# jiean001/MakeupDiffuse

Hardware: NVIDIA B200
Metric: DDIM-50 makeup images/sec at 256^2 (higher is better)
Workload: dtype bf16

## Files before the change

makeupdiffuse_b200/csrc/attention_tcgen05.cu:

```cuda
#include <cuda.h>
#include <stdlib.h>

#include "tcgen05.cuh"
using namespace mkd;
using namespace mkd::tc;

namespace {

constexpr int BQ = 128, BKV = 128;
constexpr int CH = 128 * 128;

template <int DN, int NWG_, int KST_, int VST_> struct ACfg {
  static constexpr int DCH = (DN + 63) / 64;
  static constexpr int NWG = NWG_, KST = KST_, VST = VST_;
  static constexpr int OSTR = (DN + 31) / 32 * 32;
  static constexpr int TCOLS = NWG * 128 + NWG * OSTR <= 256 ? 256 : 512;
  static constexpr int THREADS = 32 * (4 * NWG + 2);
  static constexpr int NBAR = 5 * NWG + 2 * KST + 2 * VST;
  static constexpr size_t SMEM = (size_t)(NWG * DCH + (KST + VST) * DCH + 2 * NWG) * CH + NBAR * 8 + 16;
  static_assert(NWG * 128 + NWG * OSTR <= 512, "TMEM columns");
  static_assert(SMEM <= 227 * 1024, "shared memory");
};

template <int DN, int NWG_, int KST_, int VST_>
__global__ void __launch_bounds__(ACfg<DN, NWG_, KST_, VST_>::THREADS, ACfg<DN, NWG_, KST_, VST_>::TCOLS == 256 ? 2 : 1)
    attn_tcgen05_kernel(const __grid_constant__ CUtensorMap qmap, const __grid_constant__ CUtensorMap kmap,
                        const __grid_constant__ CUtensorMap vmap, bf16* __restrict__ o, int Nq, int Nkv, int d, int ldo,
                        float sl2) {
  using C = ACfg<DN, NWG_, KST_, VST_>;
  constexpr int DCH = C::DCH, NWG = C::NWG, KST = C::KST, VST = C::VST;
  extern __shared__ __align__(1024) unsigned char smem_raw[];
  unsigned char* smem = smem_raw;
  if ((smem_u32(smem_raw) & 1023u) != 0) __trap();
  unsigned char* Qs = smem;
  unsigned char* Ks = Qs + NWG * DCH * CH;
  unsigned char* Vs = Ks + KST * DCH * CH;
  unsigned char* Ps = Vs + VST * DCH * CH;
  uint64_t* q_full = reinterpret_cast<uint64_t*>(Ps + NWG * 2 * CH);
  uint64_t* s_full = q_full + NWG;
  uint64_t* s_free = s_full + NWG;
  uint64_t* p_full = s_free + NWG;
  uint64_t* o_full = p_full + NWG;
  uint64_t* k_full = o_full + NWG;
  uint64_t* k_empty = k_full + KST;
  uint64_t* v_full = k_empty + KST;
  uint64_t* v_empty = v_full + VST;
  uint32_t* tmem_slot = reinterpret_cast<uint32_t*>(v_empty + VST);

  const int warp = threadIdx.x >> 5, lane = threadIdx.x & 31;
  constexpr int W_PROD = 4 * NWG, W_MMA = 4 * NWG + 1;
  const int b = blockIdx.z, h = blockIdx.y, q0 = blockIdx.x * (BQ * NWG);
  const int T = (Nkv + BKV - 1) / BKV;
  const int nwg = (NWG == 2 && q0 + BQ < Nq) ? 2 : 1;

  if (threadIdx.x == 0) {
    prefetch_tensormap(&qmap);
    prefetch_tensormap(&kmap);
    prefetch_tensormap(&vmap);
    for (int i = 0; i < NWG; ++i) {
      mbar_init(q_full + i, 1);
      mbar_init(s_full + i, 1);
      mbar_init(s_free + i, 4);
      mbar_init(p_full + i, 4);
      mbar_init(o_full + i, 1);
    }
    for (int i = 0; i < KST; ++i) {
      mbar_init(k_full + i, 1);
      mbar_init(k_empty + i, 1);
    }
    for (int i = 0; i < VST; ++i) {
      mbar_init(v_full + i, 1);
      mbar_init(v_empty + i, 1);
    }
    fence_barrier_init();
  }
  if (warp == W_MMA) tmem_alloc<C::TCOLS>(tmem_slot);
  fence_before();
  __syncthreads();
  fence_after();
  const uint32_t tmem_base = *tmem_slot;
  pdl_wait();
  if (warp == W_PROD) {
    if (lane == 0) {
      for (int wg = 0; wg < nwg; ++wg) {
        mbar_expect_tx(q_full + wg, DCH * CH);
        for (int c = 0; c < DCH; ++c) tma_load_4d(&qmap, q_full + wg, Qs + (wg * DCH + c) * CH, c * 64, h, q0 + wg * BQ, b);
      }
      for (int t = 0; t < T; ++t) {
        const int ks = t % KST, vs = t % VST;
        if (t >= KST) mbar_wait(k_empty + ks, (t / KST - 1) & 1);
        mbar_expect_tx(k_full + ks, DCH * CH);
        for (int c = 0; c < DCH; ++c) tma_load_4d(&kmap, k_full + ks, Ks + (ks * DCH + c) * CH, c * 64, h, t * BKV, b);
        if (t >= VST) mbar_wait(v_empty + vs, (t / VST - 1) & 1);
        mbar_expect_tx(v_full + vs, DCH * CH);
        for (int c = 0; c < DCH; ++c) tma_load_4d(&vmap, v_full + vs, Vs + (vs * DCH + c) * CH, c * 64, h, t * BKV, b);
      }
    }
  } else if (warp == W_MMA) {
    if (lane == 0) {
      constexpr uint32_t idesc_s = idesc_bf16(BQ, BKV, false);
      constexpr uint32_t idesc_o = idesc_bf16(BQ, DN, true);
      const int ksteps = (d + 15) >> 4;
      auto issue_s = [&](int wg, int st) {
        const uint32_t a = smem_u32(Qs + wg * DCH * CH), bk = smem_u32(Ks + st * DCH * CH);
        for (int ks = 0; ks < ksteps; ++ks) {
          const uint32_t off = (uint32_t)(ks >> 2) * CH + (uint32_t)(ks & 3) * 32;
          mma_bf16_ss(tmem_base + (uint32_t)(wg * BKV), smem_desc_sw128(a + off), smem_desc_sw128(bk + off), idesc_s, ks > 0);
        }
      };
      auto issue_pv = [&](int wg, int st, int kvalid, bool accumulate) {
        const uint32_t a = smem_u32(Ps + wg * 2 * CH), bv = smem_u32(Vs + st * DCH * CH);
        const int steps = (min(kvalid, BKV) + 15) >> 4;
        for (int kk = 0; kk < steps; ++kk) {
          const uint32_t aoff = (uint32_t)(kk >> 2) * CH + (uint32_t)(kk & 3) * 32;
          mma_bf16_ss(tmem_base + (uint32_t)(NWG * BKV + wg * C::OSTR), smem_desc_sw128(a + aoff),
                      smem_desc_sw128(bv + (uint32_t)kk * 2048, CH), idesc_o, accumulate || kk > 0);
        }
      };
      for (int wg = 0; wg < nwg; ++wg) mbar_wait(q_full + wg, 0);
      mbar_wait(k_full + 0, 0);
      fence_after();
      for (int wg = 0; wg < nwg; ++wg) {
        issue_s(wg, 0);
        commit(s_full + wg);
      }
      commit(k_empty + 0);
      for (int t = 0; t < T; ++t) {
        const int st = t % VST;
        if (t + 1 < T) {
          const int st1 = (t + 1) % KST;
          mbar_wait(k_full + st1, ((t + 1) / KST) & 1);
          for (int wg = 0; wg < nwg; ++wg) {
            mbar_wait(s_free + wg, t & 1);
            fence_after();
            issue_s(wg, st1);
            commit(s_full + wg);
          }
          commit(k_empty + st1);
        }
        mbar_wait(v_full + st, (t / VST) & 1);
        for (int wg = 0; wg < nwg; ++wg) {
          mbar_wait(p_full + wg, t & 1);
          fence_after();
          issue_pv(wg, st, Nkv - t * BKV, t > 0);
          commit(o_full + wg);
        }
        commit(v_empty + st);
      }
    }
  } else if ((warp >> 2) < nwg) {
    const int wg = warp >> 2, row = (warp & 3) * 32 + lane;
    const uint32_t lane_base = (uint32_t)((warp & 3) * 32) << 16;
    const uint32_t tS = tmem_base + lane_base + (uint32_t)(wg * BKV);
    const uint32_t tO = tmem_base + lane_base + (uint32_t)(NWG * BKV + wg * C::OSTR);
    unsigned char* Pw = Ps + wg * 2 * CH + row * 128;
    const uint32_t swz = (uint32_t)(row & 7);
    float m_used = -INFINITY, l = 0.f;

    for (int t = 0; t < T; ++t) {
      mbar_wait(s_full + wg, t & 1);
      fence_after();
      const int kvalid = Nkv - t * BKV;
      uint32_t v[4][32];
#pragma unroll
      for (int c = 0; c < 4; ++c) tmem_ld32_nowait(tS + c * 32, v[c]);
      tmem_ld_wait();
      fence_before();
      __syncwarp();
      if (lane == 0) mbar_arrive(s_free + wg);
      if (kvalid < BKV) {
#pragma unroll
        for (int c = 0; c < 4; ++c) {
#pragma unroll
          for (int i = 0; i < 32; ++i) v[c][i] = (c * 32 + i >= kvalid) ? 0xff800000u : v[c][i];
        }
      }
      float mx8[8];
#pragma unroll
      for (int i = 0; i < 8; ++i) mx8[i] = -INFINITY;
#pragma unroll
      for (int c = 0; c < 4; ++c) {
#pragma unroll
        for (int i = 0; i < 32; i += 2) mx8[(i >> 1) & 7] = max3(mx8[(i >> 1) & 7], __uint_as_float(v[c][i]), __uint_as_float(v[c][i + 1]));
      }
      const float mx = fmaxf(max3(mx8[0], mx8[1], mx8[2]), max3(mx8[3], mx8[4], fmaxf(max3(mx8[5], mx8[6], mx8[7]), -INFINITY)));
      if (t > 0) {
        mbar_wait(o_full + wg, (t - 1) & 1);
        fence_after();
      }
      if (__any_sync(0xffffffffu, (mx - m_used) * sl2 > 8.0f)) {
        const float m_new = fmaxf(m_used, mx);
        const float corr = ex2((m_used - m_new) * sl2);
        l *= corr;
        m_used = m_new;
        if (t > 0) {
#pragma unroll
          for (int g = 0; g < DN / 16; ++g) {
            uint32_t r[16];
            tmem_ld16_nowait(tO + g * 16, r);
            tmem_ld_wait();
#pragma unroll
            for (int i = 0; i < 16; ++i) r[i] = __float_as_uint(__uint_as_float(r[i]) * corr);
            tmem_st16(tO + g * 16, r);
          }
          tmem_st_wait();
        }
      }
      const float mb = m_used * sl2;
      const uint64_t sl2x2 = pack2(sl2, sl2), nmbx2 = pack2(-mb, -mb);
      uint64_t sum2[4] = {pack2(0.f, 0.f), pack2(0.f, 0.f), pack2(0.f, 0.f), pack2(0.f, 0.f)};
#pragma unroll
      for (int c = 0; c < 4; ++c) {
        uint32_t pk[16];
#pragma unroll
        for (int i = 0; i < 32; i += 2) {
          float a0, a1;
          unpack2(ffma2(pack2(__uint_as_float(v[c][i]), __uint_as_float(v[c][i + 1])), sl2x2, nmbx2), a0, a1);
          const float p0 = ex2(a0), p1 = ex2(a1);
          sum2[(i >> 1) & 3] = fadd2(sum2[(i >> 1) & 3], pack2(p0, p1));
          __nv_bfloat162 hh = __floats2bfloat162_rn(p0, p1);
          pk[i >> 1] = *reinterpret_cast<uint32_t*>(&hh);
        }
#pragma unroll
        for (int jj = 0; jj < 4; ++jj) {
          const uint32_t u = (uint32_t)(c * 4 + jj);
          unsigned char* dst = Pw + (u >> 3) * CH + (((u & 7) ^ swz) << 4);
          *reinterpret_cast<uint4*>(dst) = make_uint4(pk[4 * jj], pk[4 * jj + 1], pk[4 * jj + 2], pk[4 * jj + 3]);
        }
      }
      {
        float s0, s1, s2, s3;
        unpack2(fadd2(sum2[0], sum2[1]), s0, s1);
        unpack2(fadd2(sum2[2], sum2[3]), s2, s3);
        l += (s0 + s1) + (s2 + s3);
      }
      fence_before();
      fence_proxy_async_smem();
      __syncwarp();
      if (lane == 0) mbar_arrive(p_full + wg);
    }
    mbar_wait(o_full + wg, (T - 1) & 1);
    fence_after();
    const int q = q0 + wg * BQ + row;
    const float inv = 1.0f / l;
    bf16* dst = o + ((int64_t)b * Nq + q) * ldo + h * d;
#pragma unroll
    for (int g = 0; g < DN / 16; ++g) {
      uint32_t r[16];
      tmem_ld16_nowait(tO + g * 16, r);
      tmem_ld_wait();
#pragma unroll
      for (int hlf = 0; hlf < 2; ++hlf) {
        if (q < Nq && g * 16 + hlf * 8 < d) {
          float f[8];
#pragma unroll
          for (int i = 0; i < 8; ++i) f[i] = __uint_as_float(r[hlf * 8 + i]) * inv;
          store8(dst + g * 16 + hlf * 8, f);
        }
      }
    }
  }
  fence_before();
  __syncthreads();
  if (warp == W_MMA) {
    fence_after();
    tmem_dealloc<C::TCOLS>(tmem_base);
  }
}

constexpr int HKV = 64;
constexpr int HB = HKV * 128;

template <int DN>
__global__ void __launch_bounds__(320, 2)
    attn_split_kernel(const __grid_constant__ CUtensorMap qmap, const __grid_constant__ CUtensorMap kmap,
                      const __grid_constant__ CUtensorMap vmap, bf16* __restrict__ o, int Nq, int Nkv, int d, int ldo, float sl2) {
  static_assert(DN % 16 == 0 && DN <= 64, "one 64-channel chunk per head");
  constexpr int TCOLS = 256;
  extern __shared__ __align__(1024) unsigned char smem_raw[];
  unsigned char* smem = smem_raw;
  if ((smem_u32(smem_raw) & 1023u) != 0) __trap();
  unsigned char* Qs = smem;
  unsigned char* Ks = Qs + CH;
  unsigned char* Vs = Ks + 4 * HB;
  unsigned char* Ps = Vs + 4 * HB;
  uint64_t* q_full = reinterpret_cast<uint64_t*>(Ps + 2 * CH);
  uint64_t* s_full = q_full + 1;
  uint64_t* s_free = s_full + 2;
  uint64_t* p_full = s_free + 2;
  uint64_t* pv_done = p_full + 2;
  uint64_t* k_full = pv_done + 2;
  uint64_t* v_full = k_full + 4;
  uint32_t* tmem_slot = reinterpret_cast<uint32_t*>(v_full + 4);

  const int warp = threadIdx.x >> 5, lane = threadIdx.x & 31;
  constexpr int W_ISSUE = 8;
  const int b = blockIdx.z, h = blockIdx.y, q0 = blockIdx.x * BQ;
  const int H = (Nkv + HKV - 1) / HKV;

  if (threadIdx.x == 0) {
    prefetch_tensormap(&qmap);
    prefetch_tensormap(&kmap);
    prefetch_tensormap(&vmap);
    mbar_init(q_full, 1);
    for (int i = 0; i < 2; ++i) {
      mbar_init(s_full + i, 1);
      mbar_init(s_free + i, 4);
      mbar_init(p_full + i, 4);
      mbar_init(pv_done + i, 1);
    }
    for (int i = 0; i < 4; ++i) {
      mbar_init(k_full + i, 1);
      mbar_init(v_full + i, 1);
    }
    fence_barrier_init();
  }
  if (warp == W_ISSUE) tmem_alloc<TCOLS>(tmem_slot);
  fence_before();
  __syncthreads();
  fence_after();
  const uint32_t tmem_base = *tmem_slot;
  pdl_wait();
  if (warp >= W_ISSUE) {
    const int g = warp - W_ISSUE;
    const int n = (H - g + 1) >> 1;
    constexpr uint32_t idesc_s = idesc_bf16(BQ, HKV, false);
    constexpr uint32_t idesc_o = idesc_bf16(BQ, DN, true);
    constexpr int KS = DN / 16;
    unsigned char* Kg = Ks + g * 2 * HB;
    unsigned char* Vg = Vs + g * 2 * HB;
    const uint64_t qdesc = smem_desc_sw128(smem_u32(Qs));
    const uint64_t kdesc0 = smem_desc_sw128(smem_u32(Kg));
    const uint64_t vdesc0 = smem_desc_sw128(smem_u32(Vg), CH);
    const uint64_t pdesc = smem_desc_sw128(smem_u32(Ps + g * CH));
    const uint32_t dS = tmem_base + (uint32_t)(g * HKV), dO = tmem_base + (uint32_t)(2 * HKV + g * 64);
    auto load_k = [&](int u) {
      if (elect_one()) {
        mbar_expect_tx(k_full + 2 * g + (u & 1), HB);
        tma_load_4d(&kmap, k_full + 2 * g + (u & 1), Kg + (u & 1) * HB, 0, h, (g + 2 * u) * HKV, b);
      }
      __syncwarp();
    };
    auto load_v = [&](int u) {
      if (elect_one()) {
        mbar_expect_tx(v_full + 2 * g + (u & 1), HB);
        tma_load_4d(&vmap, v_full + 2 * g + (u & 1), Vg + (u & 1) * HB, 0, h, (g + 2 * u) * HKV, b);
      }
      __syncwarp();
    };
    auto issue_s = [&](int u) {
      mbar_wait(k_full + 2 * g + (u & 1), (u >> 1) & 1);
      fence_after();
      if (elect_one()) {
        const uint64_t kd = kdesc0 + (uint64_t)((u & 1) * (HB >> 4));
#pragma unroll
        for (int ks = 0; ks < KS; ++ks) mma_bf16_ss(dS, qdesc + (uint64_t)(ks * 2), kd + (uint64_t)(ks * 2), idesc_s, ks > 0);
        commit(s_full + g);
      }
      __syncwarp();
    };
    if (n > 0) {
      if (g == 0 && elect_one()) {
        mbar_expect_tx(q_full, CH);
        tma_load_4d(&qmap, q_full, Qs, 0, h, q0, b);
      }
      __syncwarp();
      load_k(0);
      load_v(0);
      if (n > 1) {
        load_k(1);
        load_v(1);
      }
      mbar_wait(q_full, 0);
      issue_s(0);
      for (int u = 0; u < n; ++u) {
        const int s = u & 1;
        if (u + 1 < n) {
          mbar_wait(s_free + g, u & 1);
          if (u + 2 < n) load_k(u + 2);
          issue_s(u + 1);
        }
        mbar_wait(v_full + 2 * g + s, (u >> 1) & 1);
        mbar_wait(p_full + g, u & 1);
        fence_after();
        if (u >= 1 && u + 1 < n) load_v(u + 1);
        if (elect_one()) {
          const uint64_t vd = vdesc0 + (uint64_t)(s * (HB >> 4));
          const int kvalid = Nkv - (g + 2 * u) * HKV;
          if (kvalid >= HKV) {
#pragma unroll
            for (int kk = 0; kk < 4; ++kk) mma_bf16_ss(dO, pdesc + (uint64_t)(kk * 2), vd + (uint64_t)(kk * 128), idesc_o, u > 0 || kk > 0);
          } else {
            const int steps = (kvalid + 15) >> 4;
            for (int kk = 0; kk < steps; ++kk) mma_bf16_ss(dO, pdesc + (uint64_t)(kk * 2), vd + (uint64_t)(kk * 128), idesc_o, u > 0 || kk > 0);
          }
          commit(pv_done + g);
        }
        __syncwarp();
      }
    }
  } else {
    const int g = warp >> 2, row = (warp & 3) * 32 + lane;
    const uint32_t lane_base = (uint32_t)((warp & 3) * 32) << 16;
    const uint32_t tS = tmem_base + lane_base + (uint32_t)(g * HKV);
    const uint32_t tO = tmem_base + lane_base + (uint32_t)(2 * HKV + g * 64);
    const uint32_t pw = smem_u32(Ps + g * CH + row * 128) + (((uint32_t)row & 7u) << 4);
    float m_used = -INFINITY, l = 0.f;
    int u = 0;
    for (int hh = g; hh < H; hh += 2, ++u) {
      mbar_wait(s_full + g, u & 1);
      fence_after();
      uint32_t v[2][32];
      tmem_ld32_nowait(tS, v[0]);
      tmem_ld32_nowait(tS + 32, v[1]);
      tmem_ld_wait();
      fence_before();
      __syncwarp();
      if (lane == 0) mbar_arrive(s_free + g);
      const int kvalid = Nkv - hh * HKV;
      if (kvalid < HKV) {
#pragma unroll
        for (int c = 0; c < 2; ++c) {
#pragma unroll
          for (int i = 0; i < 32; ++i) v[c][i] = (c * 32 + i >= kvalid) ? 0xff800000u : v[c][i];
        }
      }
      float mx8[8];
#pragma unroll
      for (int i = 0; i < 8; ++i) mx8[i] = -INFINITY;
#pragma unroll
      for (int c = 0; c < 2; ++c) {
#pragma unroll
        for (int i = 0; i < 32; i += 2) mx8[(i >> 1) & 7] = max3(mx8[(i >> 1) & 7], __uint_as_float(v[c][i]), __uint_as_float(v[c][i + 1]));
      }
      const float mx = fmaxf(max3(mx8[0], mx8[1], mx8[2]), max3(mx8[3], mx8[4], max3(mx8[5], mx8[6], mx8[7])));
      if (__any_sync(0xffffffffu, (mx - m_used) * sl2 > 8.0f)) {
        const float m_new = fmaxf(m_used, mx);
        const float corr = ex2((m_used - m_new) * sl2);
        l *= corr;
        m_used = m_new;
        if (u > 0) {
          mbar_wait(pv_done + g, (u - 1) & 1);
          fence_after();
#pragma unroll
          for (int gg = 0; gg < DN / 16; ++gg) {
            uint32_t r[16];
            tmem_ld16_nowait(tO + gg * 16, r);
            tmem_ld_wait();
#pragma unroll
            for (int i = 0; i < 16; ++i) r[i] = __float_as_uint(__uint_as_float(r[i]) * corr);
            tmem_st16(tO + gg * 16, r);
          }
          tmem_st_wait();
        }
      }
      const float mb = m_used * sl2;
      const uint64_t sl2x2 = pack2(sl2, sl2), nmbx2 = pack2(-mb, -mb);
      uint64_t sum2[4] = {pack2(0.f, 0.f), pack2(0.f, 0.f), pack2(0.f, 0.f), pack2(0.f, 0.f)};
      uint32_t pk[2][16];
#pragma unroll
      for (int c = 0; c < 2; ++c) {
#pragma unroll
        for (int i = 0; i < 32; i += 2) {
          float a0, a1;
          unpack2(ffma2(pack2(__uint_as_float(v[c][i]), __uint_as_float(v[c][i + 1])), sl2x2, nmbx2), a0, a1);
          const float p0 = ex2(a0), p1 = ex2(a1);
          sum2[(i >> 1) & 3] = fadd2(sum2[(i >> 1) & 3], pack2(p0, p1));
          __nv_bfloat162 hh2 = __floats2bfloat162_rn(p0, p1);
          pk[c][i >> 1] = *reinterpret_cast<uint32_t*>(&hh2);
        }
      }
      if (u > 0) {
        mbar_wait(pv_done + g, (u - 1) & 1);
        fence_after();
      }
#pragma unroll
      for (int c = 0; c < 2; ++c) {
#pragma unroll
        for (int jj = 0; jj < 4; ++jj)
          asm volatile("st.shared.v4.b32 [%0], {%1, %2, %3, %4};\n" ::"r"(pw ^ ((uint32_t)(c * 4 + jj) << 4)), "r"(pk[c][4 * jj]),
                       "r"(pk[c][4 * jj + 1]), "r"(pk[c][4 * jj + 2]), "r"(pk[c][4 * jj + 3])
                       : "memory");
      }
      {
        float s0, s1, s2, s3;
        unpack2(fadd2(sum2[0], sum2[1]), s0, s1);
        unpack2(fadd2(sum2[2], sum2[3]), s2, s3);
        l += (s0 + s1) + (s2 + s3);
      }
      fence_before();
      fence_proxy_async_smem();
      __syncwarp();
      if (lane == 0) mbar_arrive(p_full + g);
    }
    const bool two = H > 1;
    float2* ml = reinterpret_cast<float2*>(Ps);
    if (u > 0) {
      mbar_wait(pv_done + g, (u - 1) & 1);
      ml[g * (CH / 8) + row] = make_float2(m_used, l);
    }
    fence_before();
    asm volatile("bar.sync 1, 256;\n" ::: "memory");
    fence_after();
    const float2 mo = (g == 0 && !two) ? make_float2(-INFINITY, 0.f) : ml[(g ^ 1) * (CH / 8) + row];
    const float m = fmaxf(m_used, mo.x);
    const float a_own = ex2((m_used - m) * sl2), a_oth = ex2((mo.x - m) * sl2);
    const float inv = 1.0f / (l * a_own + mo.y * a_oth);
    const float c_own = a_own * inv, c_oth = a_oth * inv;
    const uint32_t tO_oth = tmem_base + lane_base + (uint32_t)(2 * HKV + (g ^ 1) * 64);
    const int q = q0 + row;
    bf16* dst = o + ((int64_t)b * Nq + q) * ldo + h * d;
#pragma unroll
    for (int gg = 0; gg < DN / 16; ++gg) {
      if ((gg & 1) != g) continue;
      uint32_t r0[16], r1[16];
      if (g == 0 || two) tmem_ld16_nowait(tO + gg * 16, r0);
      if (g == 1 || two) tmem_ld16_nowait(tO_oth + gg * 16, r1);
      tmem_ld_wait();
#pragma unroll
      for (int hlf = 0; hlf < 2; ++hlf) {
        if (q < Nq && gg * 16 + hlf * 8 < d) {
          float f[8];
#pragma unroll
          for (int i = 0; i < 8; ++i) {
            const float own = (g == 0 || two) ? __uint_as_float(r0[hlf * 8 + i]) * c_own : 0.f;
            const float oth = (g == 1 || two) ? __uint_as_float(r1[hlf * 8 + i]) * c_oth : 0.f;
            f[i] = own + oth;
          }
          store8(dst + gg * 16 + hlf * 8, f);
        }
      }
    }
  }
  fence_before();
  __syncthreads();
  if (warp == W_ISSUE) {
    fence_after();
    tmem_dealloc<TCOLS>(tmem_base);
  }
}

typedef CUresult (*EncodeFn)(CUtensorMap*, CUtensorMapDataType, cuuint32_t, void*, const cuuint64_t*, const cuuint64_t*,
                             const cuuint32_t*, const cuuint32_t*, CUtensorMapInterleave, CUtensorMapSwizzle,
                             CUtensorMapL2promotion, CUtensorMapFloatOOBfill);
EncodeFn get_encode() {
  static EncodeFn fn = nullptr;
  if (!fn) {
    void* p = nullptr;
    cudaDriverEntryPointQueryResult q;
    if (cudaGetDriverEntryPoint("cuTensorMapEncodeTiled", &p, cudaEnableDefault, &q) == cudaSuccess &&
        q == cudaDriverEntryPointSuccess)
      fn = reinterpret_cast<EncodeFn>(p);
  }
  return fn;
}

int head_map(CUtensorMap* map, const bf16* base, int d, int heads, int ntok, int B, int ld, int box_rows = 128) {
  cuuint64_t dims[4] = {(cuuint64_t)d, (cuuint64_t)heads, (cuuint64_t)ntok, (cuuint64_t)B};
  cuuint64_t str[3] = {(cuuint64_t)d * 2, (cuuint64_t)ld * 2, (cuuint64_t)ntok * ld * 2};
  cuuint32_t box[4] = {64, 1, (cuuint32_t)box_rows, 1};
  return tma_encode_bf16(map, base, 4, dims, str, box);
}

template <int DN, int NWG, int KST, int VST>
int launch(const bf16* q, const bf16* k, const bf16* v, bf16* o, int B, int heads, int Nq, int Nkv, int d, int ldq, int ldk,
           int ldv, int ldo, float scale, cudaStream_t st) {
  using C = ACfg<DN, NWG, KST, VST>;
  static bool configured = false;
  if (!configured) {
    cudaError_t e = cudaFuncSetAttribute(attn_tcgen05_kernel<DN, NWG, KST, VST>, cudaFuncAttributeMaxDynamicSharedMemorySize, (int)C::SMEM);
    MKD_REQUIRE(e == cudaSuccess, MKD_E_CUDA, "attention_tcgen05: cudaFuncSetAttribute(%zu): %s", C::SMEM, cudaGetErrorString(e));
    configured = true;
  }
  CUtensorMap qm, km, vm;
  int rc;
  if ((rc = head_map(&qm, q, d, heads, Nq, B, ldq))) return rc;
  if ((rc = head_map(&km, k, d, heads, Nkv, B, ldk))) return rc;
  if ((rc = head_map(&vm, v, d, heads, Nkv, B, ldv))) return rc;
  dim3 grid((Nq + BQ * C::NWG - 1) / (BQ * C::NWG), heads, B);
  MKD_LAUNCH_OK(launch_pdl(attn_tcgen05_kernel<DN, NWG, KST, VST>, grid, dim3(C::THREADS), C::SMEM, st, qm, km, vm, o, Nq, Nkv, d, ldo,
                           scale * 1.4426950408889634f));
  MKD_CHECK_LAUNCH();
  return MKD_OK;
}

template <int DN>
int launch_half(const bf16* q, const bf16* k, const bf16* v, bf16* o, int B, int heads, int Nq, int Nkv, int d, int ldq, int ldk,
                int ldv, int ldo, float scale, cudaStream_t st) {
  constexpr size_t SMEM = (size_t)7 * CH + 17 * 8 + 16;
  static_assert(2 * SMEM <= 227 * 1024, "two CTAs per SM");
  static bool configured = false;
  if (!configured) {
    cudaError_t e = cudaFuncSetAttribute(attn_split_kernel<DN>, cudaFuncAttributeMaxDynamicSharedMemorySize, (int)SMEM);
    MKD_REQUIRE(e == cudaSuccess, MKD_E_CUDA, "attention_tcgen05: cudaFuncSetAttribute(%zu): %s", SMEM, cudaGetErrorString(e));
    configured = true;
  }
  CUtensorMap qm, km, vm;
  int rc;
  if ((rc = head_map(&qm, q, d, heads, Nq, B, ldq))) return rc;
  if ((rc = head_map(&km, k, d, heads, Nkv, B, ldk, HKV))) return rc;
  if ((rc = head_map(&vm, v, d, heads, Nkv, B, ldv, HKV))) return rc;
  dim3 grid((Nq + BQ - 1) / BQ, heads, B);
  MKD_LAUNCH_OK(launch_pdl(attn_split_kernel<DN>, grid, dim3(320), SMEM, st, qm, km, vm, o, Nq, Nkv, d, ldo, scale * 1.4426950408889634f));
  MKD_CHECK_LAUNCH();
  return MKD_OK;
}
}

namespace mkd {
int tma_encode_bf16(CUtensorMap* map, const void* base, int rank, const cuuint64_t* dims, const cuuint64_t* strides_bytes,
                    const cuuint32_t* box) {
  EncodeFn fn = get_encode();
  MKD_REQUIRE(fn != nullptr, MKD_E_CUDA, "cuTensorMapEncodeTiled entry point not found (driver too old?)");
  cuuint32_t estr[5] = {1, 1, 1, 1, 1};
  CUresult r = fn(map, CU_TENSOR_MAP_DATA_TYPE_BFLOAT16, (cuuint32_t)rank, const_cast<void*>(base), dims, strides_bytes,
                  box, estr, CU_TENSOR_MAP_INTERLEAVE_NONE, CU_TENSOR_MAP_SWIZZLE_128B, CU_TENSOR_MAP_L2_PROMOTION_L2_256B,
                  CU_TENSOR_MAP_FLOAT_OOB_FILL_NONE);
  MKD_REQUIRE(r == CUDA_SUCCESS, MKD_E_CUDA, "cuTensorMapEncodeTiled failed (CUresult %d)", (int)r);
  return MKD_OK;
}

bool attention_tcgen05_supported(int d, int ldq, int ldk, int ldv) {
  return d % 8 == 0 && d >= 8 && d <= 160 && ldq % 8 == 0 && ldk % 8 == 0 && ldv % 8 == 0;
}

int attention_tcgen05(const bf16* q, const bf16* k, const bf16* v, bf16* o, int B, int heads, int Nq, int Nkv, int d,
                      int ldq, int ldk, int ldv, int ldo, float scale, cudaStream_t st) {
  const int dn = (d + 15) / 16 * 16;
  static const int whole = debug_switch("MKD_ATTN_WHOLE", 0);
#define MKD_ATTN_ARGS q, k, v, o, B, heads, Nq, Nkv, d, ldq, ldk, ldv, ldo, scale, st
  if (dn <= 64 && !whole) {
    if (dn <= 16) return launch_half<16>(MKD_ATTN_ARGS);
    if (dn <= 32) return launch_half<32>(MKD_ATTN_ARGS);
    if (dn <= 48) return launch_half<48>(MKD_ATTN_ARGS);
    return launch_half<64>(MKD_ATTN_ARGS);
  }
  if (dn <= 48) return launch<48, 1, 2, 2>(MKD_ATTN_ARGS);
  if (dn <= 64) return launch<64, 1, 2, 2>(MKD_ATTN_ARGS);
  if (dn <= 80) return launch<80, 2, 2, 1>(MKD_ATTN_ARGS);
  if (dn <= 128) return launch<128, 2, 2, 1>(MKD_ATTN_ARGS);
  return launch<160, 1, 2, 1>(MKD_ATTN_ARGS);
#undef MKD_ATTN_ARGS
}
}
```

Measured before the change: 51.55.

## Make tcgen05 attention kernels persistent with a grid-stride tile scheduler

Both attention kernels now launch one CTA per resident slot, sized by an occupancy query, and loop over (batch, head, q-tile) work items in grid-stride order. A q_empty barrier is added and all mbarrier phases carry across items, so the producer can prefetch the next tile's Q/K/V while the current tile finishes. This is meant to cut per-CTA launch, setup and TMEM allocation overhead and to overlap tile tails with the next tile's loads. In exchange the barrier phase bookkeeping gets more complex, and static round-robin assignment can leave some CTAs with uneven amounts of work.

```diff
diff --git a/makeupdiffuse_b200/csrc/attention_tcgen05.cu b/makeupdiffuse_b200/csrc/attention_tcgen05.cu
--- a/makeupdiffuse_b200/csrc/attention_tcgen05.cu
+++ b/makeupdiffuse_b200/csrc/attention_tcgen05.cu
@@ -16,7 +16,7 @@
   static constexpr int OSTR = (DN + 31) / 32 * 32;
   static constexpr int TCOLS = NWG * 128 + NWG * OSTR <= 256 ? 256 : 512;
   static constexpr int THREADS = 32 * (4 * NWG + 2);
-  static constexpr int NBAR = 5 * NWG + 2 * KST + 2 * VST;
+  static constexpr int NBAR = 6 * NWG + 2 * KST + 2 * VST;
   static constexpr size_t SMEM = (size_t)(NWG * DCH + (KST + VST) * DCH + 2 * NWG) * CH + NBAR * 8 + 16;
   static_assert(NWG * 128 + NWG * OSTR <= 512, "TMEM columns");
   static_assert(SMEM <= 227 * 1024, "shared memory");
@@ -26,7 +26,7 @@
 __global__ void __launch_bounds__(ACfg<DN, NWG_, KST_, VST_>::THREADS, ACfg<DN, NWG_, KST_, VST_>::TCOLS == 256 ? 2 : 1)
     attn_tcgen05_kernel(const __grid_constant__ CUtensorMap qmap, const __grid_constant__ CUtensorMap kmap,
                         const __grid_constant__ CUtensorMap vmap, bf16* __restrict__ o, int Nq, int Nkv, int d, int ldo,
-                        float sl2) {
+                        float sl2, int heads, int QT, int items) {
   using C = ACfg<DN, NWG_, KST_, VST_>;
   constexpr int DCH = C::DCH, NWG = C::NWG, KST = C::KST, VST = C::VST;
   extern __shared__ __align__(1024) unsigned char smem_raw[];
@@ -37,7 +37,8 @@
   unsigned char* Vs = Ks + KST * DCH * CH;
   unsigned char* Ps = Vs + VST * DCH * CH;
   uint64_t* q_full = reinterpret_cast<uint64_t*>(Ps + NWG * 2 * CH);
-  uint64_t* s_full = q_full + NWG;
+  uint64_t* q_empty = q_full + NWG;
+  uint64_t* s_full = q_empty + NWG;
   uint64_t* s_free = s_full + NWG;
   uint64_t* p_full = s_free + NWG;
   uint64_t* o_full = p_full + NWG;
@@ -49,9 +50,16 @@
 
   const int warp = threadIdx.x >> 5, lane = threadIdx.x & 31;
   constexpr int W_PROD = 4 * NWG, W_MMA = 4 * NWG + 1;
-  const int b = blockIdx.z, h = blockIdx.y, q0 = blockIdx.x * (BQ * NWG);
   const int T = (Nkv + BKV - 1) / BKV;
-  const int nwg = (NWG == 2 && q0 + BQ < Nq) ? 2 : 1;
+  const int NJ = (items - (int)blockIdx.x + (int)gridDim.x - 1) / (int)gridDim.x;
+  auto decode = [&](int it, int& b, int& h, int& q0) {
+    const int bh = it / QT;
+    q0 = (it - bh * QT) * (BQ * NWG);
+    h = bh % heads;
+    b = bh / heads;
+  };
+  auto item = [&](int j, int& b, int& h, int& q0) { decode((int)blockIdx.x + j * (int)gridDim.x, b, h, q0); };
+  auto nwg_of = [&](int q0) { return (NWG == 2 && q0 + BQ < Nq) ? 2 : 1; };
 
   if (threadIdx.x == 0) {
     prefetch_tensormap(&qmap);
@@ -59,6 +67,7 @@
     prefetch_tensormap(&vmap);
     for (int i = 0; i < NWG; ++i) {
       mbar_init(q_full + i, 1);
+      mbar_init(q_empty + i, 1);
       mbar_init(s_full + i, 1);
       mbar_init(s_free + i, 4);
       mbar_init(p_full + i, 4);
@@ -82,18 +91,28 @@
   pdl_wait();
   if (warp == W_PROD) {
     if (lane == 0) {
-      for (int wg = 0; wg < nwg; ++wg) {
-        mbar_expect_tx(q_full + wg, DCH * CH);
-        for (int c = 0; c < DCH; ++c) tma_load_4d(&qmap, q_full + wg, Qs + (wg * DCH + c) * CH, c * 64, h, q0 + wg * BQ, b);
-      }
-      for (int t = 0; t < T; ++t) {
-        const int ks = t % KST, vs = t % VST;
-        if (t >= KST) mbar_wait(k_empty + ks, (t / KST - 1) & 1);
-        mbar_expect_tx(k_full + ks, DCH * CH);
-        for (int c = 0; c < DCH; ++c) tma_load_4d(&kmap, k_full + ks, Ks + (ks * DCH + c) * CH, c * 64, h, t * BKV, b);
-        if (t >= VST) mbar_wait(v_empty + vs, (t / VST - 1) & 1);
-        mbar_expect_tx(v_full + vs, DCH * CH);
-        for (int c = 0; c < DCH; ++c) tma_load_4d(&vmap, v_full + vs, Vs + (vs * DCH + c) * CH, c * 64, h, t * BKV, b);
+      int qi[NWG] = {};
+      for (int j = 0, kt = 0; j < NJ; ++j, kt += T) {
+        int b, h, q0;
+        item(j, b, h, q0);
+        const int nwg = nwg_of(q0);
+#pragma unroll
+        for (int wg = 0; wg < NWG; ++wg) {
+          if (wg >= nwg) continue;
+          if (qi[wg] > 0) mbar_wait(q_empty + wg, (qi[wg] - 1) & 1);
+          ++qi[wg];
+          mbar_expect_tx(q_full + wg, DCH * CH);
+          for (int c = 0; c < DCH; ++c) tma_load_4d(&qmap, q_full + wg, Qs + (wg * DCH + c) * CH, c * 64, h, q0 + wg * BQ, b);
+        }
+        for (int t = 0; t < T; ++t) {
+          const int n = kt + t, ks = n % KST, vs = n % VST;
+          if (n >= KST) mbar_wait(k_empty + ks, (n / KST - 1) & 1);
+          mbar_expect_tx(k_full + ks, DCH * CH);
+          for (int c = 0; c < DCH; ++c) tma_load_4d(&kmap, k_full + ks, Ks + (ks * DCH + c) * CH, c * 64, h, t * BKV, b);
+          if (n >= VST) mbar_wait(v_empty + vs, (n / VST - 1) & 1);
+          mbar_expect_tx(v_full + vs, DCH * CH);
+          for (int c = 0; c < DCH; ++c) tma_load_4d(&vmap, v_full + vs, Vs + (vs * DCH + c) * CH, c * 64, h, t * BKV, b);
+        }
       }
     }
   } else if (warp == W_MMA) {
@@ -117,147 +136,172 @@
                       smem_desc_sw128(bv + (uint32_t)kk * 2048, CH), idesc_o, accumulate || kk > 0);
         }
       };
-      for (int wg = 0; wg < nwg; ++wg) mbar_wait(q_full + wg, 0);
-      mbar_wait(k_full + 0, 0);
-      fence_after();
-      for (int wg = 0; wg < nwg; ++wg) {
-        issue_s(wg, 0);
-        commit(s_full + wg);
-      }
-      commit(k_empty + 0);
-      for (int t = 0; t < T; ++t) {
-        const int st = t % VST;
-        if (t + 1 < T) {
-          const int st1 = (t + 1) % KST;
-          mbar_wait(k_full + st1, ((t + 1) / KST) & 1);
-          for (int wg = 0; wg < nwg; ++wg) {
-            mbar_wait(s_free + wg, t & 1);
+      int qi[NWG] = {};
+      for (int j = 0, kt = 0; j < NJ; ++j, kt += T) {
+        int b, h, q0;
+        item(j, b, h, q0);
+        const int nwg = nwg_of(q0);
+        mbar_wait(k_full + kt % KST, (kt / KST) & 1);
+#pragma unroll
+        for (int wg = 0; wg < NWG; ++wg) {
+          if (wg >= nwg) continue;
+          mbar_wait(q_full + wg, qi[wg] & 1);
+          if (qi[wg] > 0) mbar_wait(s_free + wg, (qi[wg] * T - 1) & 1);
+          fence_after();
+          issue_s(wg, kt % KST);
+          commit(s_full + wg);
+          if (T == 1) commit(q_empty + wg);
+        }
+        commit(k_empty + kt % KST);
+        for (int t = 0; t < T; ++t) {
+          const int n = kt + t, st = n % VST;
+          if (t + 1 < T) {
+            const int st1 = (n + 1) % KST;
+            mbar_wait(k_full + st1, ((n + 1) / KST) & 1);
+#pragma unroll
+            for (int wg = 0; wg < NWG; ++wg) {
+              if (wg >= nwg) continue;
+              mbar_wait(s_free + wg, (qi[wg] * T + t) & 1);
+              fence_after();
+              issue_s(wg, st1);
+              commit(s_full + wg);
+              if (t + 2 == T) commit(q_empty + wg);
+            }
+            commit(k_empty + st1);
+          }
+          mbar_wait(v_full + st, (n / VST) & 1);
+#pragma unroll
+          for (int wg = 0; wg < NWG; ++wg) {
+            if (wg >= nwg) continue;
+            mbar_wait(p_full + wg, (qi[wg] * T + t) & 1);
             fence_after();
-            issue_s(wg, st1);
-            commit(s_full + wg);
-          }
-          commit(k_empty + st1);
-        }
-        mbar_wait(v_full + st, (t / VST) & 1);
-        for (int wg = 0; wg < nwg; ++wg) {
-          mbar_wait(p_full + wg, t & 1);
-          fence_after();
-          issue_pv(wg, st, Nkv - t * BKV, t > 0);
-          commit(o_full + wg);
-        }
-        commit(v_empty + st);
-      }
-    }
-  } else if ((warp >> 2) < nwg) {
+            issue_pv(wg, st, Nkv - t * BKV, t > 0);
+            commit(o_full + wg);
+          }
+          commit(v_empty + st);
+        }
+#pragma unroll
+        for (int wg = 0; wg < NWG; ++wg) qi[wg] += wg < nwg ? 1 : 0;
+      }
+    }
+  } else if (warp < W_PROD) {
     const int wg = warp >> 2, row = (warp & 3) * 32 + lane;
     const uint32_t lane_base = (uint32_t)((warp & 3) * 32) << 16;
     const uint32_t tS = tmem_base + lane_base + (uint32_t)(wg * BKV);
     const uint32_t tO = tmem_base + lane_base + (uint32_t)(NWG * BKV + wg * C::OSTR);
     unsigned char* Pw = Ps + wg * 2 * CH + row * 128;
     const uint32_t swz = (uint32_t)(row & 7);
-    float m_used = -INFINITY, l = 0.f;
-
-    for (int t = 0; t < T; ++t) {
-      mbar_wait(s_full + wg, t & 1);
+    for (int it = blockIdx.x, n0 = 0; it < items; it += gridDim.x) {
+      int b, h, q0;
+      decode(it, b, h, q0);
+      if (wg >= nwg_of(q0)) continue;
+      b = h = q0 = 0;
+      float m_used = -INFINITY, l = 0.f;
+
+      for (int t = 0; t < T; ++t) {
+        mbar_wait(s_full + wg, (n0 + t) & 1);
+        fence_after();
+        const int kvalid = Nkv - t * BKV;
+        uint32_t v[4][32];
+#pragma unroll
+        for (int c = 0; c < 4; ++c) tmem_ld32_nowait(tS + c * 32, v[c]);
+        tmem_ld_wait();
+        fence_before();
+        __syncwarp();
+        if (lane == 0) mbar_arrive(s_free + wg);
+        if (kvalid < BKV) {
+#pragma unroll
+          for (int c = 0; c < 4; ++c) {
+#pragma unroll
+            for (int i = 0; i < 32; ++i) v[c][i] = (c * 32 + i >= kvalid) ? 0xff800000u : v[c][i];
+          }
+        }
+        float mx8[8];
+#pragma unroll
+        for (int i = 0; i < 8; ++i) mx8[i] = -INFINITY;
+#pragma unroll
+        for (int c = 0; c < 4; ++c) {
+#pragma unroll
+          for (int i = 0; i < 32; i += 2) mx8[(i >> 1) & 7] = max3(mx8[(i >> 1) & 7], __uint_as_float(v[c][i]), __uint_as_float(v[c][i + 1]));
+        }
+        const float mx = fmaxf(max3(mx8[0], mx8[1], mx8[2]), max3(mx8[3], mx8[4], fmaxf(max3(mx8[5], mx8[6], mx8[7]), -INFINITY)));
+        if (t > 0) {
+          mbar_wait(o_full + wg, (n0 + t - 1) & 1);
+          fence_after();
+        }
+        if (__any_sync(0xffffffffu, (mx - m_used) * sl2 > 8.0f)) {
+          const float m_new = fmaxf(m_used, mx);
+          const float corr = ex2((m_used - m_new) * sl2);
+          l *= corr;
+          m_used = m_new;
+          if (t > 0) {
+#pragma unroll
+            for (int g = 0; g < DN / 16; ++g) {
+              uint32_t r[16];
+              tmem_ld16_nowait(tO + g * 16, r);
+              tmem_ld_wait();
+#pragma unroll
+              for (int i = 0; i < 16; ++i) r[i] = __float_as_uint(__uint_as_float(r[i]) * corr);
+              tmem_st16(tO + g * 16, r);
+            }
+            tmem_st_wait();
+          }
+        }
+        const float mb = m_used * sl2;
+        const uint64_t sl2x2 = pack2(sl2, sl2), nmbx2 = pack2(-mb, -mb);
+        uint64_t sum2[4] = {pack2(0.f, 0.f), pack2(0.f, 0.f), pack2(0.f, 0.f), pack2(0.f, 0.f)};
+#pragma unroll
+        for (int c = 0; c < 4; ++c) {
+          uint32_t pk[16];
+#pragma unroll
+          for (int i = 0; i < 32; i += 2) {
+            float a0, a1;
+            unpack2(ffma2(pack2(__uint_as_float(v[c][i]), __uint_as_float(v[c][i + 1])), sl2x2, nmbx2), a0, a1);
+            const float p0 = ex2(a0), p1 = ex2(a1);
+            sum2[(i >> 1) & 3] = fadd2(sum2[(i >> 1) & 3], pack2(p0, p1));
+            __nv_bfloat162 hh = __floats2bfloat162_rn(p0, p1);
+            pk[i >> 1] = *reinterpret_cast<uint32_t*>(&hh);
+          }
+#pragma unroll
+          for (int jj = 0; jj < 4; ++jj) {
+            const uint32_t u = (uint32_t)(c * 4 + jj);
+            unsigned char* dst = Pw + (u >> 3) * CH + (((u & 7) ^ swz) << 4);
+            *reinterpret_cast<uint4*>(dst) = make_uint4(pk[4 * jj], pk[4 * jj + 1], pk[4 * jj + 2], pk[4 * jj + 3]);
+          }
+        }
+        {
+          float s0, s1, s2, s3;
+          unpack2(fadd2(sum2[0], sum2[1]), s0, s1);
+          unpack2(fadd2(sum2[2], sum2[3]), s2, s3);
+          l += (s0 + s1) + (s2 + s3);
+        }
+        fence_before();
+        fence_proxy_async_smem();
+        __syncwarp();
+        if (lane == 0) mbar_arrive(p_full + wg);
+      }
+      mbar_wait(o_full + wg, (n0 + T - 1) & 1);
       fence_after();
-      const int kvalid = Nkv - t * BKV;
-      uint32_t v[4][32];
-#pragma unroll
-      for (int c = 0; c < 4; ++c) tmem_ld32_nowait(tS + c * 32, v[c]);
-      tmem_ld_wait();
-      fence_before();
-      __syncwarp();
-      if (lane == 0) mbar_arrive(s_free + wg);
-      if (kvalid < BKV) {
-#pragma unroll
-        for (int c = 0; c < 4; ++c) {
-#pragma unroll
-          for (int i = 0; i < 32; ++i) v[c][i] = (c * 32 + i >= kvalid) ? 0xff800000u : v[c][i];
-        }
-      }
-      float mx8[8];
-#pragma unroll
-      for (int i = 0; i < 8; ++i) mx8[i] = -INFINITY;
-#pragma unroll
-      for (int c = 0; c < 4; ++c) {
-#pragma unroll
-        for (int i = 0; i < 32; i += 2) mx8[(i >> 1) & 7] = max3(mx8[(i >> 1) & 7], __uint_as_float(v[c][i]), __uint_as_float(v[c][i + 1]));
-      }
-      const float mx = fmaxf(max3(mx8[0], mx8[1], mx8[2]), max3(mx8[3], mx8[4], fmaxf(max3(mx8[5], mx8[6], mx8[7]), -INFINITY)));
-      if (t > 0) {
-        mbar_wait(o_full + wg, (t - 1) & 1);
-        fence_after();
-      }
-      if (__any_sync(0xffffffffu, (mx - m_used) * sl2 > 8.0f)) {
-        const float m_new = fmaxf(m_used, mx);
-        const float corr = ex2((m_used - m_new) * sl2);
-        l *= corr;
-        m_used = m_new;
-        if (t > 0) {
-#pragma unroll
-          for (int g = 0; g < DN / 16; ++g) {
-            uint32_t r[16];
-            tmem_ld16_nowait(tO + g * 16, r);
-            tmem_ld_wait();
-#pragma unroll
-            for (int i = 0; i < 16; ++i) r[i] = __float_as_uint(__uint_as_float(r[i]) * corr);
-            tmem_st16(tO + g * 16, r);
-          }
-          tmem_st_wait();
-        }
-      }
-      const float mb = m_used * sl2;
-      const uint64_t sl2x2 = pack2(sl2, sl2), nmbx2 = pack2(-mb, -mb);
-      uint64_t sum2[4] = {pack2(0.f, 0.f), pack2(0.f, 0.f), pack2(0.f, 0.f), pack2(0.f, 0.f)};
-#pragma unroll
-      for (int c = 0; c < 4; ++c) {
-        uint32_t pk[16];
-#pragma unroll
-        for (int i = 0; i < 32; i += 2) {
-          float a0, a1;
-          unpack2(ffma2(pack2(__uint_as_float(v[c][i]), __uint_as_float(v[c][i + 1])), sl2x2, nmbx2), a0, a1);
-          const float p0 = ex2(a0), p1 = ex2(a1);
-          sum2[(i >> 1) & 3] = fadd2(sum2[(i >> 1) & 3], pack2(p0, p1));
-          __nv_bfloat162 hh = __floats2bfloat162_rn(p0, p1);
-          pk[i >> 1] = *reinterpret_cast<uint32_t*>(&hh);
-        }
-#pragma unroll
-        for (int jj = 0; jj < 4; ++jj) {
-          const uint32_t u = (uint32_t)(c * 4 + jj);
-          unsigned char* dst = Pw + (u >> 3) * CH + (((u & 7) ^ swz) << 4);
-          *reinterpret_cast<uint4*>(dst) = make_uint4(pk[4 * jj], pk[4 * jj + 1], pk[4 * jj + 2], pk[4 * jj + 3]);
-        }
-      }
-      {
-        float s0, s1, s2, s3;
-        unpack2(fadd2(sum2[0], sum2[1]), s0, s1);
-        unpack2(fadd2(sum2[2], sum2[3]), s2, s3);
-        l += (s0 + s1) + (s2 + s3);
-      }
-      fence_before();
-      fence_proxy_async_smem();
-      __syncwarp();
-      if (lane == 0) mbar_arrive(p_full + wg);
-    }
-    mbar_wait(o_full + wg, (T - 1) & 1);
-    fence_after();
-    const int q = q0 + wg * BQ + row;
-    const float inv = 1.0f / l;
-    bf16* dst = o + ((int64_t)b * Nq + q) * ldo + h * d;
-#pragma unroll
-    for (int g = 0; g < DN / 16; ++g) {
-      uint32_t r[16];
-      tmem_ld16_nowait(tO + g * 16, r);
-      tmem_ld_wait();
-#pragma unroll
-      for (int hlf = 0; hlf < 2; ++hlf) {
-        if (q < Nq && g * 16 + hlf * 8 < d) {
-          float f[8];
-#pragma unroll
-          for (int i = 0; i < 8; ++i) f[i] = __uint_as_float(r[hlf * 8 + i]) * inv;
-          store8(dst + g * 16 + hlf * 8, f);
-        }
-      }
+      decode(it, b, h, q0);
+      const int q = q0 + wg * BQ + row;
+      const float inv = 1.0f / l;
+      bf16* dst = o + ((int64_t)b * Nq + q) * ldo + h * d;
+#pragma unroll
+      for (int g = 0; g < DN / 16; ++g) {
+        uint32_t r[16];
+        tmem_ld16_nowait(tO + g * 16, r);
+        tmem_ld_wait();
+#pragma unroll
+        for (int hlf = 0; hlf < 2; ++hlf) {
+          if (q < Nq && g * 16 + hlf * 8 < d) {
+            float f[8];
+#pragma unroll
+            for (int i = 0; i < 8; ++i) f[i] = __uint_as_float(r[hlf * 8 + i]) * inv;
+            store8(dst + g * 16 + hlf * 8, f);
+          }
+        }
+      }
+      n0 += T;
     }
   }
   fence_before();
@@ -274,7 +318,8 @@
 template <int DN>
 __global__ void __launch_bounds__(320, 2)
     attn_split_kernel(const __grid_constant__ CUtensorMap qmap, const __grid_constant__ CUtensorMap kmap,
-                      const __grid_constant__ CUtensorMap vmap, bf16* __restrict__ o, int Nq, int Nkv, int d, int ldo, float sl2) {
+                      const __grid_constant__ CUtensorMap vmap, bf16* __restrict__ o, int Nq, int Nkv, int d, int ldo, float sl2,
+                      int heads, int QT, int items) {
   static_assert(DN % 16 == 0 && DN <= 64, "one 64-channel chunk per head");
   constexpr int TCOLS = 256;
   extern __shared__ __align__(1024) unsigned char smem_raw[];
@@ -285,7 +330,8 @@
   unsigned char* Vs = Ks + 4 * HB;
   unsigned char* Ps = Vs + 4 * HB;
   uint64_t* q_full = reinterpret_cast<uint64_t*>(Ps + 2 * CH);
-  uint64_t* s_full = q_full + 1;
+  uint64_t* q_empty = q_full + 1;
+  uint64_t* s_full = q_empty + 1;
   uint64_t* s_free = s_full + 2;
   uint64_t* p_full = s_free + 2;
   uint64_t* pv_done = p_full + 2;
@@ -295,14 +341,22 @@
 
   const int warp = threadIdx.x >> 5, lane = threadIdx.x & 31;
   constexpr int W_ISSUE = 8;
-  const int b = blockIdx.z, h = blockIdx.y, q0 = blockIdx.x * BQ;
   const int H = (Nkv + HKV - 1) / HKV;
+  const int NJ = (items - (int)blockIdx.x + (int)gridDim.x - 1) / (int)gridDim.x;
+  auto decode = [&](int it, int& b, int& h, int& q0) {
+    const int bh = it / QT;
+    q0 = (it - bh * QT) * BQ;
+    h = bh % heads;
+    b = bh / heads;
+  };
+  auto item = [&](int j, int& b, int& h, int& q0) { decode((int)blockIdx.x + j * (int)gridDim.x, b, h, q0); };
 
   if (threadIdx.x == 0) {
     prefetch_tensormap(&qmap);
     prefetch_tensormap(&kmap);
     prefetch_tensormap(&vmap);
     mbar_init(q_full, 1);
+    mbar_init(q_empty, H > 1 ? 2 : 1);
     for (int i = 0; i < 2; ++i) {
       mbar_init(s_full + i, 1);
       mbar_init(s_free + i, 4);
@@ -324,6 +378,7 @@
   if (warp >= W_ISSUE) {
     const int g = warp - W_ISSUE;
     const int n = (H - g + 1) >> 1;
+    const int total = NJ * n;
     constexpr uint32_t idesc_s = idesc_bf16(BQ, HKV, false);
     constexpr uint32_t idesc_o = idesc_bf16(BQ, DN, true);
     constexpr int KS = DN / 16;
@@ -334,56 +389,62 @@
     const uint64_t vdesc0 = smem_desc_sw128(smem_u32(Vg), CH);
     const uint64_t pdesc = smem_desc_sw128(smem_u32(Ps + g * CH));
     const uint32_t dS = tmem_base + (uint32_t)(g * HKV), dO = tmem_base + (uint32_t)(2 * HKV + g * 64);
-    auto load_k = [&](int u) {
+    auto load_kv = [&](const CUtensorMap* map, uint64_t* full, unsigned char* ring, int c) {
+      int b, h, q0;
+      item(c / n, b, h, q0);
       if (elect_one()) {
-        mbar_expect_tx(k_full + 2 * g + (u & 1), HB);
-        tma_load_4d(&kmap, k_full + 2 * g + (u & 1), Kg + (u & 1) * HB, 0, h, (g + 2 * u) * HKV, b);
+        mbar_expect_tx(full + 2 * g + (c & 1), HB);
+        tma_load_4d(map, full + 2 * g + (c & 1), ring + (c & 1) * HB, 0, h, (g + 2 * (c % n)) * HKV, b);
       }
       __syncwarp();
     };
-    auto load_v = [&](int u) {
+    auto load_k = [&](int c) { load_kv(&kmap, k_full, Kg, c); };
+    auto load_v = [&](int c) { load_kv(&vmap, v_full, Vg, c); };
+    auto load_q = [&](int j) {
+      int b, h, q0;
+      item(j, b, h, q0);
       if (elect_one()) {
-        mbar_expect_tx(v_full + 2 * g + (u & 1), HB);
-        tma_load_4d(&vmap, v_full + 2 * g + (u & 1), Vg + (u & 1) * HB, 0, h, (g + 2 * u) * HKV, b);
+        mbar_expect_tx(q_full, CH);
+        tma_load_4d(&qmap, q_full, Qs, 0, h, q0, b);
       }
       __syncwarp();
     };
-    auto issue_s = [&](int u) {
-      mbar_wait(k_full + 2 * g + (u & 1), (u >> 1) & 1);
+    auto issue_s = [&](int c) {
+      mbar_wait(k_full + 2 * g + (c & 1), (c >> 1) & 1);
       fence_after();
       if (elect_one()) {
-        const uint64_t kd = kdesc0 + (uint64_t)((u & 1) * (HB >> 4));
+        const uint64_t kd = kdesc0 + (uint64_t)((c & 1) * (HB >> 4));
 #pragma unroll
         for (int ks = 0; ks < KS; ++ks) mma_bf16_ss(dS, qdesc + (uint64_t)(ks * 2), kd + (uint64_t)(ks * 2), idesc_s, ks > 0);
         commit(s_full + g);
+        if (c % n == n - 1) commit(q_empty);
       }
       __syncwarp();
     };
     if (n > 0) {
-      if (g == 0 && elect_one()) {
-        mbar_expect_tx(q_full, CH);
-        tma_load_4d(&qmap, q_full, Qs, 0, h, q0, b);
-      }
-      __syncwarp();
+      if (g == 0) load_q(0);
       load_k(0);
       load_v(0);
-      if (n > 1) {
+      if (total > 1) {
         load_k(1);
         load_v(1);
       }
       mbar_wait(q_full, 0);
       issue_s(0);
-      for (int u = 0; u < n; ++u) {
-        const int s = u & 1;
+      for (int c = 0, j = 0, u = 0; c < total; ++c) {
+        const int s = c & 1;
         if (u + 1 < n) {
-          mbar_wait(s_free + g, u & 1);
-          if (u + 2 < n) load_k(u + 2);
-          issue_s(u + 1);
-        }
-        mbar_wait(v_full + 2 * g + s, (u >> 1) & 1);
-        mbar_wait(p_full + g, u & 1);
+          mbar_wait(s_free + g, c & 1);
+          if (c + 2 < total) load_k(c + 2);
+          issue_s(c + 1);
+        } else if (g == 0 && j + 1 < NJ) {
+          mbar_wait(q_empty, j & 1);
+          load_q(j + 1);
+        }
+        mbar_wait(v_full + 2 * g + s, (c >> 1) & 1);
+        mbar_wait(p_full + g, c & 1);
         fence_after();
-        if (u >= 1 && u + 1 < n) load_v(u + 1);
+        if (c >= 1 && c + 1 < total) load_v(c + 1);
         if (elect_one()) {
           const uint64_t vd = vdesc0 + (uint64_t)(s * (HB >> 4));
           const int kvalid = Nkv - (g + 2 * u) * HKV;
@@ -397,6 +458,16 @@
           commit(pv_done + g);
         }
         __syncwarp();
+        if (u + 1 == n && j + 1 < NJ) {
+          mbar_wait(s_free + g, c & 1);
+          if (c + 2 < total) load_k(c + 2);
+          mbar_wait(q_full, (j + 1) & 1);
+          issue_s(c + 1);
+        }
+        if (++u == n) {
+          u = 0;
+          ++j;
+        }
       }
     }
   } else {
@@ -405,131 +476,136 @@
     const uint32_t tS = tmem_base + lane_base + (uint32_t)(g * HKV);
     const uint32_t tO = tmem_base + lane_base + (uint32_t)(2 * HKV + g * 64);
     const uint32_t pw = smem_u32(Ps + g * CH + row * 128) + (((uint32_t)row & 7u) << 4);
-    float m_used = -INFINITY, l = 0.f;
-    int u = 0;
-    for (int hh = g; hh < H; hh += 2, ++u) {
-      mbar_wait(s_full + g, u & 1);
+    for (int it = blockIdx.x, hs = 0; it < items; it += gridDim.x) {
+      float m_used = -INFINITY, l = 0.f;
+      int u = 0;
+      for (int hh = g; hh < H; hh += 2, ++u, ++hs) {
+        mbar_wait(s_full + g, hs & 1);
+        fence_after();
+        uint32_t v[2][32];
+        tmem_ld32_nowait(tS, v[0]);
+        tmem_ld32_nowait(tS + 32, v[1]);
+        tmem_ld_wait();
+        fence_before();
+        __syncwarp();
+        if (lane == 0) mbar_arrive(s_free + g);
+        const int kvalid = Nkv - hh * HKV;
+        if (kvalid < HKV) {
+#pragma unroll
+          for (int c = 0; c < 2; ++c) {
+#pragma unroll
+            for (int i = 0; i < 32; ++i) v[c][i] = (c * 32 + i >= kvalid) ? 0xff800000u : v[c][i];
+          }
+        }
+        float mx8[8];
+#pragma unroll
+        for (int i = 0; i < 8; ++i) mx8[i] = -INFINITY;
+#pragma unroll
+        for (int c = 0; c < 2; ++c) {
+#pragma unroll
+          for (int i = 0; i < 32; i += 2) mx8[(i >> 1) & 7] = max3(mx8[(i >> 1) & 7], __uint_as_float(v[c][i]), __uint_as_float(v[c][i + 1]));
+        }
+        const float mx = fmaxf(max3(mx8[0], mx8[1], mx8[2]), max3(mx8[3], mx8[4], max3(mx8[5], mx8[6], mx8[7])));
+        if (__any_sync(0xffffffffu, (mx - m_used) * sl2 > 8.0f)) {
+          const float m_new = fmaxf(m_used, mx);
+          const float corr = ex2((m_used - m_new) * sl2);
+          l *= corr;
+          m_used = m_new;
+          if (u > 0) {
+            mbar_wait(pv_done + g, (hs - 1) & 1);
+            fence_after();
+#pragma unroll
+            for (int gg = 0; gg < DN / 16; ++gg) {
+              uint32_t r[16];
+              tmem_ld16_nowait(tO + gg * 16, r);
+              tmem_ld_wait();
+#pragma unroll
+              for (int i = 0; i < 16; ++i) r[i] = __float_as_uint(__uint_as_float(r[i]) * corr);
+              tmem_st16(tO + gg * 16, r);
+            }
+            tmem_st_wait();
+          }
+        }
+        const float mb = m_used * sl2;
+        const uint64_t sl2x2 = pack2(sl2, sl2), nmbx2 = pack2(-mb, -mb);
+        uint64_t sum2[4] = {pack2(0.f, 0.f), pack2(0.f, 0.f), pack2(0.f, 0.f), pack2(0.f, 0.f)};
+        uint32_t pk[2][16];
+#pragma unroll
+        for (int c = 0; c < 2; ++c) {
+#pragma unroll
+          for (int i = 0; i < 32; i += 2) {
+            float a0, a1;
+            unpack2(ffma2(pack2(__uint_as_float(v[c][i]), __uint_as_float(v[c][i + 1])), sl2x2, nmbx2), a0, a1);
+            const float p0 = ex2(a0), p1 = ex2(a1);
+            sum2[(i >> 1) & 3] = fadd2(sum2[(i >> 1) & 3], pack2(p0, p1));
+            __nv_bfloat162 hh2 = __floats2bfloat162_rn(p0, p1);
+            pk[c][i >> 1] = *reinterpret_cast<uint32_t*>(&hh2);
+          }
+        }
+        if (u > 0) {
+          mbar_wait(pv_done + g, (hs - 1) & 1);
+          fence_after();
+        }
+#pragma unroll
+        for (int c = 0; c < 2; ++c) {
+#pragma unroll
+          for (int jj = 0; jj < 4; ++jj)
+            asm volatile("st.shared.v4.b32 [%0], {%1, %2, %3, %4};\n" ::"r"(pw ^ ((uint32_t)(c * 4 + jj) << 4)), "r"(pk[c][4 * jj]),
+                         "r"(pk[c][4 * jj + 1]), "r"(pk[c][4 * jj + 2]), "r"(pk[c][4 * jj + 3])
+                         : "memory");
+        }
+        {
+          float s0, s1, s2, s3;
+          unpack2(fadd2(sum2[0], sum2[1]), s0, s1);
+          unpack2(fadd2(sum2[2], sum2[3]), s2, s3);
+          l += (s0 + s1) + (s2 + s3);
+        }
+        fence_before();
+        fence_proxy_async_smem();
+        __syncwarp();
+        if (lane == 0) mbar_arrive(p_full + g);
+      }
+      const bool two = H > 1;
+      float2* ml = reinterpret_cast<float2*>(Ps);
+      if (u > 0) {
+        mbar_wait(pv_done + g, (hs - 1) & 1);
+        ml[g * (CH / 8) + row] = make_float2(m_used, l);
+      }
+      fence_before();
+      asm volatile("bar.sync 1, 256;\n" ::: "memory");
       fence_after();
-      uint32_t v[2][32];
-      tmem_ld32_nowait(tS, v[0]);
-      tmem_ld32_nowait(tS + 32, v[1]);
-      tmem_ld_wait();
+      const float2 mo = (g == 0 && !two) ? make_float2(-INFINITY, 0.f) : ml[(g ^ 1) * (CH / 8) + row];
+      const float m = fmaxf(m_used, mo.x);
+      const float a_own = ex2((m_used - m) * sl2), a_oth = ex2((mo.x - m) * sl2);
+      const float inv = 1.0f / (l * a_own + mo.y * a_oth);
+      const float c_own = a_own * inv, c_oth = a_oth * inv;
+      const uint32_t tO_oth = tmem_base + lane_base + (uint32_t)(2 * HKV + (g ^ 1) * 64);
+      int b, h, q0;
+      decode(it, b, h, q0);
+      const int q = q0 + row;
+      bf16* dst = o + ((int64_t)b * Nq + q) * ldo + h * d;
+      for (int gg = g; gg < DN / 16; gg += 2) {
+        uint32_t r0[16], r1[16];
+        if (g == 0 || two) tmem_ld16_nowait(tO + gg * 16, r0);
+        if (g == 1 || two) tmem_ld16_nowait(tO_oth + gg * 16, r1);
+        tmem_ld_wait();
+#pragma unroll
+        for (int hlf = 0; hlf < 2; ++hlf) {
+          if (q < Nq && gg * 16 + hlf * 8 < d) {
+            float f[8];
+#pragma unroll
+            for (int i = 0; i < 8; ++i) {
+              const float own = (g == 0 || two) ? __uint_as_float(r0[hlf * 8 + i]) * c_own : 0.f;
+              const float oth = (g == 1 || two) ? __uint_as_float(r1[hlf * 8 + i]) * c_oth : 0.f;
+              f[i] = own + oth;
+            }
+            store8(dst + gg * 16 + hlf * 8, f);
+          }
+        }
+      }
       fence_before();
-      __syncwarp();
-      if (lane == 0) mbar_arrive(s_free + g);
-      const int kvalid = Nkv - hh * HKV;
-      if (kvalid < HKV) {
-#pragma unroll
-        for (int c = 0; c < 2; ++c) {
-#pragma unroll
-          for (int i = 0; i < 32; ++i) v[c][i] = (c * 32 + i >= kvalid) ? 0xff800000u : v[c][i];
-        }
-      }
-      float mx8[8];
-#pragma unroll
-      for (int i = 0; i < 8; ++i) mx8[i] = -INFINITY;
-#pragma unroll
-      for (int c = 0; c < 2; ++c) {
-#pragma unroll
-        for (int i = 0; i < 32; i += 2) mx8[(i >> 1) & 7] = max3(mx8[(i >> 1) & 7], __uint_as_float(v[c][i]), __uint_as_float(v[c][i + 1]));
-      }
-      const float mx = fmaxf(max3(mx8[0], mx8[1], mx8[2]), max3(mx8[3], mx8[4], max3(mx8[5], mx8[6], mx8[7])));
-      if (__any_sync(0xffffffffu, (mx - m_used) * sl2 > 8.0f)) {
-        const float m_new = fmaxf(m_used, mx);
-        const float corr = ex2((m_used - m_new) * sl2);
-        l *= corr;
-        m_used = m_new;
-        if (u > 0) {
-          mbar_wait(pv_done + g, (u - 1) & 1);
-          fence_after();
-#pragma unroll
-          for (int gg = 0; gg < DN / 16; ++gg) {
-            uint32_t r[16];
-            tmem_ld16_nowait(tO + gg * 16, r);
-            tmem_ld_wait();
-#pragma unroll
-            for (int i = 0; i < 16; ++i) r[i] = __float_as_uint(__uint_as_float(r[i]) * corr);
-            tmem_st16(tO + gg * 16, r);
-          }
-          tmem_st_wait();
-        }
-      }
-      const float mb = m_used * sl2;
-      const uint64_t sl2x2 = pack2(sl2, sl2), nmbx2 = pack2(-mb, -mb);
-      uint64_t sum2[4] = {pack2(0.f, 0.f), pack2(0.f, 0.f), pack2(0.f, 0.f), pack2(0.f, 0.f)};
-      uint32_t pk[2][16];
-#pragma unroll
-      for (int c = 0; c < 2; ++c) {
-#pragma unroll
-        for (int i = 0; i < 32; i += 2) {
-          float a0, a1;
-          unpack2(ffma2(pack2(__uint_as_float(v[c][i]), __uint_as_float(v[c][i + 1])), sl2x2, nmbx2), a0, a1);
-          const float p0 = ex2(a0), p1 = ex2(a1);
-          sum2[(i >> 1) & 3] = fadd2(sum2[(i >> 1) & 3], pack2(p0, p1));
-          __nv_bfloat162 hh2 = __floats2bfloat162_rn(p0, p1);
-          pk[c][i >> 1] = *reinterpret_cast<uint32_t*>(&hh2);
-        }
-      }
-      if (u > 0) {
-        mbar_wait(pv_done + g, (u - 1) & 1);
-        fence_after();
-      }
-#pragma unroll
-      for (int c = 0; c < 2; ++c) {
-#pragma unroll
-        for (int jj = 0; jj < 4; ++jj)
-          asm volatile("st.shared.v4.b32 [%0], {%1, %2, %3, %4};\n" ::"r"(pw ^ ((uint32_t)(c * 4 + jj) << 4)), "r"(pk[c][4 * jj]),
-                       "r"(pk[c][4 * jj + 1]), "r"(pk[c][4 * jj + 2]), "r"(pk[c][4 * jj + 3])
-                       : "memory");
-      }
-      {
-        float s0, s1, s2, s3;
-        unpack2(fadd2(sum2[0], sum2[1]), s0, s1);
-        unpack2(fadd2(sum2[2], sum2[3]), s2, s3);
-        l += (s0 + s1) + (s2 + s3);
-      }
-      fence_before();
-      fence_proxy_async_smem();
-      __syncwarp();
-      if (lane == 0) mbar_arrive(p_full + g);
-    }
-    const bool two = H > 1;
-    float2* ml = reinterpret_cast<float2*>(Ps);
-    if (u > 0) {
-      mbar_wait(pv_done + g, (u - 1) & 1);
-      ml[g * (CH / 8) + row] = make_float2(m_used, l);
-    }
-    fence_before();
-    asm volatile("bar.sync 1, 256;\n" ::: "memory");
-    fence_after();
-    const float2 mo = (g == 0 && !two) ? make_float2(-INFINITY, 0.f) : ml[(g ^ 1) * (CH / 8) + row];
-    const float m = fmaxf(m_used, mo.x);
-    const float a_own = ex2((m_used - m) * sl2), a_oth = ex2((mo.x - m) * sl2);
-    const float inv = 1.0f / (l * a_own + mo.y * a_oth);
-    const float c_own = a_own * inv, c_oth = a_oth * inv;
-    const uint32_t tO_oth = tmem_base + lane_base + (uint32_t)(2 * HKV + (g ^ 1) * 64);
-    const int q = q0 + row;
-    bf16* dst = o + ((int64_t)b * Nq + q) * ldo + h * d;
-#pragma unroll
-    for (int gg = 0; gg < DN / 16; ++gg) {
-      if ((gg & 1) != g) continue;
-      uint32_t r0[16], r1[16];
-      if (g == 0 || two) tmem_ld16_nowait(tO + gg * 16, r0);
-      if (g == 1 || two) tmem_ld16_nowait(tO_oth + gg * 16, r1);
-      tmem_ld_wait();
-#pragma unroll
-      for (int hlf = 0; hlf < 2; ++hlf) {
-        if (q < Nq && gg * 16 + hlf * 8 < d) {
-          float f[8];
-#pragma unroll
-          for (int i = 0; i < 8; ++i) {
-            const float own = (g == 0 || two) ? __uint_as_float(r0[hlf * 8 + i]) * c_own : 0.f;
-            const float oth = (g == 1 || two) ? __uint_as_float(r1[hlf * 8 + i]) * c_oth : 0.f;
-            f[i] = own + oth;
-          }
-          store8(dst + gg * 16 + hlf * 8, f);
-        }
-      }
+      asm volatile("bar.sync 1, 256;\n" ::: "memory");
+      fence_after();
     }
   }
   fence_before();
@@ -562,24 +638,33 @@
   return tma_encode_bf16(map, base, 4, dims, str, box);
 }
 
+template <typename K> int resident_ctas(K kernel, int threads, size_t smem, int* out) {
+  int occ = 0;
+  cudaError_t e = cudaOccupancyMaxActiveBlocksPerMultiprocessor(&occ, kernel, threads, smem);
+  MKD_REQUIRE(e == cudaSuccess && occ > 0, MKD_E_CUDA, "attention_tcgen05: occupancy query failed: %s", cudaGetErrorString(e));
+  *out = occ * num_sms();
+  return MKD_OK;
+}
+
 template <int DN, int NWG, int KST, int VST>
 int launch(const bf16* q, const bf16* k, const bf16* v, bf16* o, int B, int heads, int Nq, int Nkv, int d, int ldq, int ldk,
            int ldv, int ldo, float scale, cudaStream_t st) {
   using C = ACfg<DN, NWG, KST, VST>;
-  static bool configured = false;
-  if (!configured) {
+  static int resident = 0;
+  if (!resident) {
     cudaError_t e = cudaFuncSetAttribute(attn_tcgen05_kernel<DN, NWG, KST, VST>, cudaFuncAttributeMaxDynamicSharedMemorySize, (int)C::SMEM);
     MKD_REQUIRE(e == cudaSuccess, MKD_E_CUDA, "attention_tcgen05: cudaFuncSetAttribute(%zu): %s", C::SMEM, cudaGetErrorString(e));
-    configured = true;
+    const int rc = resident_ctas(attn_tcgen05_kernel<DN, NWG, KST, VST>, C::THREADS, C::SMEM, &resident);
+    if (rc) return rc;
   }
   CUtensorMap qm, km, vm;
   int rc;
   if ((rc = head_map(&qm, q, d, heads, Nq, B, ldq))) return rc;
   if ((rc = head_map(&km, k, d, heads, Nkv, B, ldk))) return rc;
   if ((rc = head_map(&vm, v, d, heads, Nkv, B, ldv))) return rc;
-  dim3 grid((Nq + BQ * C::NWG - 1) / (BQ * C::NWG), heads, B);
-  MKD_LAUNCH_OK(launch_pdl(attn_tcgen05_kernel<DN, NWG, KST, VST>, grid, dim3(C::THREADS), C::SMEM, st, qm, km, vm, o, Nq, Nkv, d, ldo,
-                           scale * 1.4426950408889634f));
+  const int qtiles = (Nq + BQ * C::NWG - 1) / (BQ * C::NWG), items = qtiles * heads * B;
+  MKD_LAUNCH_OK(launch_pdl(attn_tcgen05_kernel<DN, NWG, KST, VST>, dim3(min(items, resident)), dim3(C::THREADS), C::SMEM, st, qm, km, vm,
+                           o, Nq, Nkv, d, ldo, scale * 1.4426950408889634f, heads, qtiles, items));
   MKD_CHECK_LAUNCH();
   return MKD_OK;
 }
@@ -587,21 +672,23 @@
 template <int DN>
 int launch_half(const bf16* q, const bf16* k, const bf16* v, bf16* o, int B, int heads, int Nq, int Nkv, int d, int ldq, int ldk,
                 int ldv, int ldo, float scale, cudaStream_t st) {
-  constexpr size_t SMEM = (size_t)7 * CH + 17 * 8 + 16;
+  constexpr size_t SMEM = (size_t)7 * CH + 18 * 8 + 16;
   static_assert(2 * SMEM <= 227 * 1024, "two CTAs per SM");
-  static bool configured = false;
-  if (!configured) {
+  static int resident = 0;
+  if (!resident) {
     cudaError_t e = cudaFuncSetAttribute(attn_split_kernel<DN>, cudaFuncAttributeMaxDynamicSharedMemorySize, (int)SMEM);
     MKD_REQUIRE(e == cudaSuccess, MKD_E_CUDA, "attention_tcgen05: cudaFuncSetAttribute(%zu): %s", SMEM, cudaGetErrorString(e));
-    configured = true;
+    const int rc = resident_ctas(attn_split_kernel<DN>, 320, SMEM, &resident);
+    if (rc) return rc;
   }
   CUtensorMap qm, km, vm;
   int rc;
   if ((rc = head_map(&qm, q, d, heads, Nq, B, ldq))) return rc;
   if ((rc = head_map(&km, k, d, heads, Nkv, B, ldk, HKV))) return rc;
   if ((rc = head_map(&vm, v, d, heads, Nkv, B, ldv, HKV))) return rc;
-  dim3 grid((Nq + BQ - 1) / BQ, heads, B);
-  MKD_LAUNCH_OK(launch_pdl(attn_split_kernel<DN>, grid, dim3(320), SMEM, st, qm, km, vm, o, Nq, Nkv, d, ldo, scale * 1.4426950408889634f));
+  const int qtiles = (Nq + BQ - 1) / BQ, items = qtiles * heads * B;
+  MKD_LAUNCH_OK(launch_pdl(attn_split_kernel<DN>, dim3(min(items, resident)), dim3(320), SMEM, st, qm, km, vm, o, Nq, Nkv, d, ldo,
+                           scale * 1.4426950408889634f, heads, qtiles, items));
   MKD_CHECK_LAUNCH();
   return MKD_OK;
 }
```

New measurement: 46.69, median of 6. -9.4%, worse.
